# tux550/RayTracer-RPF

Hardware: AMD Instinct MI355X
Metric: RPF Msamples/sec filtered at 1080p×8spp (higher is better)
Workload: dtype f64

## Files before the change

### raytracer-rpf_amd/csrc/rpf_api.hip

```cpp
#include <hip/hip_runtime.h>
#include <dlfcn.h>

#include <chrono>
#include <climits>
#include <cmath>
#include <cstdio>
#include <cstdlib>
#include <cstring>
#include <string>
#include <thread>
#include <vector>

#include "rpf_internal.h"

using namespace rpf;

struct rpf_ctx {
    int device = 0;
    hipStream_t stream = nullptr;
    std::string err;
    char *d_planes = nullptr;    size_t cap_planes = 0;
    float *d_rayw = nullptr;     size_t cap_rayw = 0;
    double *d_colA = nullptr;    size_t cap_colA = 0;
    double *d_colB = nullptr;    size_t cap_colB = 0;
// ... 123 lines not shown
int32_t ensure_tables(rpf_ctx *ctx, int nmax) {
    if (ctx->d_tfix && ctx->tfix_n >= nmax + 1) return RPF_OK;
    std::vector<uint64_t> t((size_t)nmax + 1), d((size_t)nmax + 1, 0);
    t[0] = 0;
    for (int k = 1; k <= nmax; ++k) t[k] = (uint64_t)std::llroundl(std::ldexp((long double)k * std::log((long double)k), 44));
    for (int k = 0; k < nmax; ++k) d[k] = t[k + 1] - t[k];
    int32_t st;
    if ((st = ensure(ctx, ctx->d_tfix, ctx->cap_tfix, t.size() * sizeof(uint64_t)))) return st;
    if ((st = ensure(ctx, ctx->d_dfix, ctx->cap_dfix, d.size() * sizeof(uint64_t)))) return st;
    HIP_TRY(hipMemcpy(ctx->d_tfix, t.data(), t.size() * sizeof(uint64_t), hipMemcpyHostToDevice));
    HIP_TRY(hipMemcpy(ctx->d_dfix, d.data(), d.size() * sizeof(uint64_t), hipMemcpyHostToDevice));
    ctx->tfix_n = nmax + 1;
    return RPF_OK;
}

struct PassSetup {
    PassParams p;
    uint32_t lds = 0;
};

int32_t setup_pass(rpf_ctx *ctx, const rpf_desc *d, int box, const void *d_planes, const double *col_in,
                   double *col_out, const rpf_debug *dbg_dev, PassSetup &out) {
    if (box < 1 || (box & 1) == 0) return fail(ctx, RPF_E_BADARG, "box must be odd and positive");
    PassParams &p = out.p;
    std::memset(&p, 0, sizeof(p));
    p.W = d->W; p.H = d->H; p.S = d->S;
    p.lay = layout_of(d);
    const int kNFeat = p.lay.nF;
    p.row_begin = d->row_begin; p.row_end = d->row_end;
    p.box = box; p.b = (box - 1) / 2;
    p.beta_map = d->beta_map; p.policy = d->degenerate_policy;
    p.fast_weights = (d->flags & RPF_FLAG_FAST_WEIGHTS) ? 1 : 0;
    p.stage_mask = ctx->tun.stage_mask;
    p.screen = ctx->tun.screen;
    const int64_t nmax64 = (int64_t)box * box * d->S;
    if (nmax64 > kMaxNbhd) return fail(ctx, RPF_E_UNSUPPORTED, "box*box*S > 65535: neighbourhood too large (16-bit histogram cells, one-byte bin ids)");
    p.nmax = (int)nmax64;
    {
        const int64_t per_px = (int64_t)box * d->S * 88;
        const int64_t budget = d->S > 8 ? (256 << 10) : (1 << 20);
        int w = (int)(budget / std::max<int64_t>(per_px, 1)) - 2 * ((box - 1) / 2);
        w = std::max(8, std::min(128, w));
        p.strip_w = w & ~7;
        if (ctx->tun.strip_w > 0) p.strip_w = ctx->tun.strip_w;
    }
    p.bmax = (int)std::sqrt((double)p.nmax);
    if (p.bmax < 1) p.bmax = 1;
    p.eps = d->eps; p.seed = d->sigma_seed;
    p.sigma_p = (double)(box / 4);
    p.plane_stride = (uint64_t)d->W * d->H * d->S;
    p.planes = d_planes; p.col_in = col_in; p.col_out = col_out;
    const size_t HW = (size_t)d->W * d->H;
    int32_t st;
    if ((st = ensure(ctx, ctx->d_pmean, ctx->cap_pmean, HW * kNFeat * sizeof(double)))) return st;
    if ((st = ensure(ctx, ctx->d_pstd, ctx->cap_pstd, HW * kNFeat * sizeof(double)))) return st;
    if ((st = ensure(ctx, ctx->d_nbhd, ctx->cap_nbhd, HW * sizeof(int32_t)))) return st;
    if ((st = ensure_tables(ctx, p.nmax))) return st;
    p.pmean = ctx->d_pmean; p.pstd = ctx->d_pstd; p.tfix = ctx->d_tfix; p.dfix = ctx->d_dfix;
    p.nbhd = ctx->d_nbhd; p.status = ctx->d_status;
    if ((st = ensure(ctx, ctx->d_flat, ctx->cap_flat, HW))) return st;
    p.flat = ctx->d_flat; p.nan_flag = ctx->d_nan_flag;
    if (dbg_dev) p.dbg = *dbg_dev;
    {
        const int nres = std::min(p.nmax, kMaxResident), bres = std::max(1, (int)std::sqrt((double)nres));
        out.lds = lds_layout(p.S, nres, bres, table_in_lds(p.S, nres, bres, ctx->tun, p.lay), ctx->tun, p.lay).total;
    }
    if ((int)out.lds > max_lds_per_block())
// ... 590 lines not shown
    HIP_TRY(hipSetDevice(ctx->device));
    hipStream_t s = (hipStream_t)stream;
    return run_passes(ctx, d, d_planes, d_colour, s);
}

int32_t rpf_host_alloc(rpf_ctx *ctx, uint64_t bytes, void **out) {
    if (!ctx) return RPF_E_BADARG;
    if (!out) return fail(ctx, RPF_E_BADARG, "out is NULL");
    *out = nullptr;
    HIP_TRY(hipSetDevice(ctx->device));
    hipError_t e = hipHostMalloc(out, bytes ? (size_t)bytes : 16, hipHostMallocDefault);
    if (e != hipSuccess)
        return fail(ctx, e == hipErrorOutOfMemory ? RPF_E_NOMEM : RPF_E_HIP, std::string("hipHostMalloc: ") + hipGetErrorString(e));
    return RPF_OK;
}

int32_t rpf_host_free(rpf_ctx *ctx, void *ptr) {
    if (!ptr) return RPF_OK;
    const hipError_t e = hipHostFree(ptr);
    if (e != hipSuccess) return fail(ctx, RPF_E_HIP, std::string("hipHostFree: ") + hipGetErrorString(e));
    return RPF_OK;
}

int32_t rpf_set_option(rpf_ctx *ctx, const char *name, int64_t value) {
    if (!ctx) return RPF_E_BADARG;
    if (!name) return fail(ctx, RPF_E_BADARG, "option name is NULL");
    const std::string n(name);
    Tuning &t = ctx->tun;
    if (n == "stage_mask") t.stage_mask = (int32_t)value;
    else if (n == "binning" && value >= -1 && value <= 1) t.binning = (int32_t)value;
    else if (n == "waves_per_pixel" && (value == 0 || value == 1 || value == 4)) t.waves_per_pixel = (int32_t)value;
    else if (n == "table_in_lds" && value >= -1 && value <= 1) t.table_in_lds = (int32_t)value;
    else if (n == "screen" && value >= 0 && value <= 1) t.screen = (int32_t)value;
    else if (n == "split_weights" && value >= -1 && value <= 1) t.split_weights = (int32_t)value;
    else if (n == "strip_w" && value >= 0 && value <= 4096 && value % 8 == 0) t.strip_w = (int32_t)value;
    else if (n == "packed" && value >= -1 && value <= 1) t.packed = (int32_t)value;
    else if (n == "split_chunk" && value >= 0 && value <= (1 << 30)) t.split_chunk = (int32_t)value;
    else if (n == "count_first" && value >= -1 && value <= 1) t.count_first = (int32_t)value;
    else if (n == "lds_pad" && value >= 0 && value <= 160 * 1024) t.lds_pad = (int32_t)value;
    else return fail(ctx, RPF_E_BADARG, "unknown option or value out of range: " + n);
    ctx->bin_valid = false;
    return RPF_OK;
}

int32_t rpf_filter(rpf_ctx *ctx, const rpf_desc *d, const void *planes, const float *ray_weight,
                   float *sample_rgb_out, float *pixel_rgb_out) {
    return rpf_filter_ex(ctx, d, planes, nullptr, ray_weight, sample_rgb_out, pixel_rgb_out, nullptr);
}

int32_t rpf_filter_ex(rpf_ctx *ctx, const rpf_desc *d, const void *planes, const double *colour64_in,
                      const float *ray_weight, float *sample_rgb_out, float *pixel_rgb_out, double *colour64_out) {
    int32_t st = validate(ctx, d, true);
    if (st) return st;
    if (!planes) return fail(ctx, RPF_E_BADARG, "planes is NULL");
    HIP_TRY(hipSetDevice(ctx->device));
    hipStream_t s = ctx->stream;
    const size_t ps = (size_t)d->W * d->H * d->S, HW = (size_t)d->W * d->H;
    const SampleLayout lay = layout_of(d);
    const size_t plane_total = (size_t)lay.ndim() * ps * lay.plane_bytes();
    if ((st = ensure(ctx, ctx->d_planes, ctx->cap_planes, plane_total))) return st;
    if ((st = ensure(ctx, ctx->d_colA, ctx->cap_colA, 3 * ps * sizeof(double)))) return st;
    if (ray_weight && (st = ensure(ctx, ctx->d_rayw, ctx->cap_rayw, ps * sizeof(float)))) return st;
    if (sample_rgb_out && (st = ensure(ctx, ctx->d_srgb, ctx->cap_srgb, 3 * ps * sizeof(float)))) return st;
    if (pixel_rgb_out && (st = ensure(ctx, ctx->d_prgb, ctx->cap_prgb, 3 * HW * sizeof(float)))) return st;
    auto pinned = [](const void *p) {
        if (!p) return true;
// ... 567 lines not shown
```

### raytracer-rpf_amd/csrc/rpf_filter_impl.inc

```

constexpr int kNR = RPF_IMPL_NR;
constexpr int kNFeat = RPF_IMPL_NF;
constexpr int kColP = 0, kColC = 2, kColR = 5, kColF = 5 + kNR;
constexpr int kNDim = 5 + kNR + kNFeat;
constexpr int kNX = kNDim - 3;
constexpr int kNAnc = kNR + 2;
constexpr int kNPairF = kNFeat * kNAnc;
constexpr int kNPairC = kNAnc + kNFeat;
constexpr int kNPair = kNPairF + 3 * kNPairC;
#ifndef RPF_ROWS_EARLY
#define RPF_ROWS_EARLY 1
#endif
constexpr int kNWt = 5 + kNFeat;
constexpr bool kRef19 = (kNR == 2 && kNFeat == 12);
using plane_t = RPF_IMPL_PLANE_T;
static_assert(kNDim <= 32 && kNFeat <= 32, "lane maps: one chain lane per column inside a 32-lane half");

__host__ __device__ constexpr int xcol(int i) { return i < 2 ? i : i + 3; }
__device__ __forceinline__ float ldp(const PassParams &p, int col, uint32_t off) {
    return (float)reinterpret_cast<const plane_t *>(p.planes)[(uint64_t)col * p.plane_stride + off];
}
__device__ __forceinline__ void pair_cols(int pr, int &ca, int &cb) {
    if (pr < kNPairF) {
        const int i = pr / kNAnc, l = pr - i * kNAnc;
        ca = kColF + i;
        cb = l < kNR ? kColR + l : kColP + (l - kNR);
    } else {
        const int q = pr - kNPairF, c = q / kNPairC, l = q - c * kNPairC;
        ca = kColC + c;
        cb = l < kNR ? kColR + l : (l < kNAnc ? kColP + (l - kNR) : kColF + (l - kNAnc));
    }
}
__device__ __forceinline__ int pair_index_of(int a, int i) {
    return a < kNAnc ? (i < kNFeat ? i * kNAnc + a : kNPairF + (i - kNFeat) * kNPairC + a)
                     : kNPairF + (a - kNAnc) * kNPairC + kNAnc + i;
}
__device__ __forceinline__ int anchor_col(int a) { return a < kNR ? kColR + a : (a < kNAnc ? kColP + (a - kNR) : kColC + (a - kNAnc)); }

__device__ __forceinline__ double load_col(const PassParams &p, int c, uint32_t off) {
    if (c >= kColC && c < kColC + 3) return p.col_in[(uint64_t)(c - kColC) * p.plane_stride + off];
    return (double)ldp(p, c, off);
}
// ... 83 lines not shown
            if (KD > 12) reinterpret_cast<uint8_t *>(sBinW + kNDim * kWave * KW)[c * kWave + lane] = (uint8_t)b.b6;
        }
    }
}
template <int KD, int KW, int PACK5>
__device__ __forceinline__ void load_bins(const uint32_t *sBinW, int c, int lane, BinIds<KW, PACK5> &b) {
    if constexpr (PACK5 == 1) {
        b.w[0] = sBinW[c * kWave + lane];
        b.b6 = (KD > 6) ? (uint32_t) reinterpret_cast<const uint8_t *>(sBinW + kNDim * kWave)[c * kWave + lane] : 0u;
    } else {
        load_words<KW>(sBinW + ((size_t)c * kWave + lane) * KW, b.w);
        b.b6 = 0u;
        if constexpr (PACK5 == 7) {
            if (KD > 12) b.b6 = (uint32_t) reinterpret_cast<const uint8_t *>(sBinW + kNDim * kWave * KW)[c * kWave + lane];
        }
    }
}
template <int KW, int PACK5>
__device__ __forceinline__ uint32_t bin_of_sample(const uint32_t *sBinW, int c, int j) {
    const int ln = j & 63, slot = j >> 6;
    if constexpr (PACK5 == 1) {
        if (slot < 6) return (sBinW[c * kWave + ln] >> (5 * slot)) & 31u;
        return reinterpret_cast<const uint8_t *>(sBinW + kNDim * kWave)[c * kWave + ln];
    } else if constexpr (PACK5 == 7) {
        if (slot < 12) return (sBinW[((size_t)c * kWave + ln) * KW + slot / 6] >> (5 * (slot % 6))) & 31u;
        return reinterpret_cast<const uint8_t *>(sBinW + kNDim * kWave * KW)[c * kWave + ln];
    } else {
        constexpr int BITS = PACK5 == 6 ? 6 : 5, SPW = 32 / BITS;
        return (sBinW[((size_t)c * kWave + ln) * KW + slot / SPW] >> (BITS * (slot % SPW))) & ((1u << BITS) - 1u);
    }
}

constexpr int kColConst = 5;
__device__ __forceinline__ void column_constants(const double *sStat, double *sCK, int c) {
    const double Mc = sStat[c], SDc = sStat[kNDim + c];
    const double xlo = sStat[2 * kNDim + c], xhi = sStat[3 * kNDim + c];
    const bool sd0 = (SDc == 0.0);
    const UDiv dsd = udiv_prepare(SDc);
    const double lo = sd0 ? 0.0 : udiv(xlo - Mc, dsd);
    const double hi = sd0 ? 0.0 : udiv(xhi - Mc, dsd);
    const double range = hi - lo;
    const bool flat = !(hi != lo);
    const UDiv drg = udiv_prepare(range);
    const bool fast = dsd.fast && (flat || drg.fast);
    double *ck = sCK + c * kColConst;
    ck[0] = dsd.r; ck[1] = lo; ck[2] = range; ck[3] = drg.r;
    ck[4] = (double)((sd0 ? 1 : 0) | (flat ? 2 : 0) | (fast ? 4 : 0));
}

template <int KD, int KW, int PACK5, int NW = 1>
__device__ __forceinline__ void bins_stage(const PassParams &p, const double *sStat, const uint32_t *sOff, uint32_t *sBinW,
                                           int lane, int n, int B, const double *sCK, int wv = 0) {
    const double dB = (double)B;
    {
        uint32_t offk[KD];
#pragma unroll
        for (int kk = 0; kk < KD; ++kk) offk[kk] = (lane + kWave * kk < n) ? sOff[lane + kWave * kk] : 0u;
        auto do_column = [&](int c, const double (&xv)[KD]) {
            const double Mc = sStat[c], SDc = sStat[kNDim + c];
            const double *ck = sCK + c * kColConst;
            const double lo = ck[1], range = ck[2];
            const int flags = (int)ck[4];
            const bool sd0 = flags & 1, flat = flags & 2, fast = flags & 4;
            UDiv dsd, drg;
            dsd.b = SDc; dsd.r = ck[0]; dsd.fast = true;
            drg.b = range; drg.r = ck[3]; drg.fast = true;
            BinIds<KW, PACK5> w;
            w.clear();
            if (sd0 || flat) {
            } else if (fast) {
#pragma unroll
                for (int kk = 0; kk < KD; ++kk) {
                    const double a = xv[kk] - Mc;
                    const double z = udiv_fast(a, dsd);
                    const double t = udiv_fast(z - lo, drg) * dB;
                    int bin = (int)t;
                    bin = min(bin, B - 1);
                    bin = max(bin, 0);
                    bin = (lane + kWave * kk < n) ? bin : 0;
                    w.set(kk, (uint32_t)bin);
                }
            } else {
#pragma unroll
                for (int kk = 0; kk < KD; ++kk) {
                    if (lane + kWave * kk < n) {
                        const double a = xv[kk] - Mc;
                        const double z = sd0 ? 0.0 : a / SDc;
                        int bin = 0;
                        if (!flat) {
                            const double t = (z - lo) / range * dB;
                            bin = (int)t;
                            bin = min(bin, B - 1);
                            bin = max(bin, 0);
                        }
                        w.set(kk, (uint32_t)bin);
                    }
                }
            }
            store_bins<KD, KW, PACK5>(sBinW, c, lane, w);
        };
        if constexpr (NW > 1) {
            if (p.stage_mask & 2) {
                auto colidx = [](int i) { return xcol(i); };
                float xb[KD];
                auto issue3 = [&](int i) {
                    const plane_t *fplane = reinterpret_cast<const plane_t *>(p.planes) + (uint64_t)colidx(i) * p.plane_stride;
#pragma unroll
                    for (int kk = 0; kk < KD; ++kk) xb[kk] = (float)fplane[offk[kk]];
                };
                issue3(wv);
#pragma unroll 1
                for (int i = wv; i < kNX; i += NW) {
                    double xv[KD];
#pragma unroll
                    for (int kk = 0; kk < KD; ++kk) xv[kk] = (double)xb[kk];
                    if (i + NW < kNX) issue3(i + NW);
                    do_column(colidx(i), xv);
                }
#pragma unroll 1
                for (int c = wv; c < 3; c += NW) {
                    double xc[KD];
                    const double *dplane = p.col_in + (uint64_t)c * p.plane_stride;
#pragma unroll
                    for (int kk = 0; kk < KD; ++kk) xc[kk] = dplane[offk[kk]];
                    do_column(kColC + c, xc);
                }
            }
        } else if (p.stage_mask & 2) {
            constexpr int kPF3 = KD <= 8 ? 4 : (KD <= 13 ? 2 : 1);
            static_assert(kNX % 4 == 0, "the column loop below walks whole groups of kPF3");
            float xb[kPF3][KD];
            auto colidx = [](int i) { return xcol(i); };
            auto issue3 = [&](int i, float (&dst)[KD]) {
                const plane_t *fplane = reinterpret_cast<const plane_t *>(p.planes) + (uint64_t)colidx(i) * p.plane_stride;
#pragma unroll
                for (int kk = 0; kk < KD; ++kk) dst[kk] = (float)fplane[offk[kk]];
            };
#pragma unroll
            for (int u = 0; u < kPF3; ++u) issue3(u, xb[u]);
#pragma unroll 1
            for (int i0 = 0; i0 < kNX; i0 += kPF3) {
#pragma unroll
                for (int u = 0; u < kPF3; ++u) {
                    double xv[KD];
#pragma unroll
                    for (int kk = 0; kk < KD; ++kk) xv[kk] = (double)xb[u][kk];
                    if (i0 + u + kPF3 < kNX) issue3(i0 + u + kPF3, xb[u]);
                    do_column(colidx(i0 + u), xv);
                }
            }
            double xc[3][KD];
#pragma unroll
            for (int c = 0; c < 3; ++c) {
                const double *dplane = p.col_in + (uint64_t)c * p.plane_stride;
#pragma unroll
                for (int kk = 0; kk < KD; ++kk) xc[c][kk] = dplane[offk[kk]];
            }
#pragma unroll
            for (int c = 0; c < 3; ++c) do_column(kColC + c, xc[c]);
        }
    }
}

template <int NIT, bool ROWS>
__device__ __forceinline__ uint32_t marginal_counts(const uint32_t *sHist, int lane, int B) {
    uint32_t tot = 0u;
    const int j = lane & 31, h = lane >> 5;
    uint32_t v[NIT];
    if constexpr (!ROWS) {
        const uint32_t *col = sHist + h * B + j;
#pragma unroll
        for (int t = 0; t < NIT; ++t) v[t] = col[2 * t * B];
#pragma unroll
        for (int t = 0; t < NIT; ++t) tot += v[t];
    } else {
        const int jj = min(j, B - 1);
#pragma unroll
        for (int t = 0; t < NIT; ++t) v[t] = sHist[jj * B + min(2 * t + h, B - 1)];
#pragma unroll
// ... 835 lines not shown
                    for (int i = 0; i < 3; ++i) vd[i] = p.col_in[(uint64_t)i * p.plane_stride + off];
                }
            };
            fetch(lane);
            for (int j0 = 0; j0 < nrun; j0 += kStageChunk) {
                const int cnt = min(kStageChunk, nrun - j0);
                if (lane < cnt) {
#pragma unroll
                    for (int i = 0; i < kNX; ++i) {
                        fmn[i] = fminf(fmn[i], vf[i]);
                        fmx[i] = fmaxf(fmx[i], vf[i]);
                    }
#pragma unroll
                    for (int i = 0; i < 3; ++i) {
                        cmn[i] = fmin(cmn[i], vd[i]);
                        cmx[i] = fmax(cmx[i], vd[i]);
                    }
                    if (j0 + lane < S) {
#pragma unroll
                        for (int i = 0; i < kNX; ++i) sOwn[(j0 + lane) * kNDim + xcol(i)] = (double)vf[i];
#pragma unroll
                        for (int i = 0; i < 3; ++i) sOwn[(j0 + lane) * kNDim + kColC + i] = vd[i];
                    }
                }
#pragma unroll
                for (int hf = 0; hf < 2; ++hf) {
                    const int cnth = min(kStageHalf, cnt - hf * kStageHalf);
                    const int t = lane - hf * kStageHalf;
                    if (t >= 0 && t < cnth) {
#pragma unroll
                        for (int i = 0; i < kNX; ++i) sStage[xcol(i) * (kStageHalf + 1) + t] = (double)vf[i];
#pragma unroll
                        for (int i = 0; i < 3; ++i) sStage[(kColC + i) * (kStageHalf + 1) + t] = vd[i];
                    }
                    wsync();
                    if (hf == 1) fetch(j0 + kStageChunk + lane);
                    if (chain && cnth > 0) {
                        const double *src = sStage + myc * (kStageHalf + 1);
                        if (cnth == kStageHalf) {
#pragma unroll
                            for (int h = 0; h < kStageHalf; h += 16) {
                                double v[16];
#pragma unroll
                                for (int q = 0; q < 16; ++q) v[q] = src[h + q];
#pragma unroll
                                for (int q = 0; q < 16; ++q) v[q] = is_sq ? v[q] * v[q] : v[q];
#pragma unroll
                                for (int q = 0; q < 16; ++q) acc = acc + v[q];
                            }
                        } else if (!is_sq) {
                            for (int q = 0; q < cnth; ++q) acc = acc + src[q];
                        } else {
                            for (int q = 0; q < cnth; ++q) { const double v = src[q]; acc = acc + v * v; }
                        }
                    }
                    wsync();
                }
            }
            const double sq = __shfl(acc, (lane & 31) + 32, 64);
            const double dn = (double)n;
            const double mean = acc / dn;
            double sd = sqrt(sq / dn - mean * mean);
            if (p.policy == RPF_DEGEN_EPS && isnan(sd)) sd = 0.0;
            if (lane < kNDim) {
                sStat[lane] = mean;
                sStat[kNDim + lane] = sd;
                if (p.dbg.mean) p.dbg.mean[pix * kNDim + lane] = mean;
                if (p.dbg.stddev) p.dbg.stddev[pix * kNDim + lane] = sd;
            }
            {
                wave_minmax(fmn, fmx, lane, sStat + 2 * kNDim, sStat + 3 * kNDim);
#pragma unroll
                for (int i = 0; i < 3; ++i) {
                    const double lo = xl::allreduce<xl::OpMin>(cmn[i]), hi = xl::allreduce<xl::OpMax>(cmx[i]);
                    if (lane == 0) { sStat[2 * kNDim + kColC + i] = lo; sStat[3 * kNDim + kColC + i] = hi; }
                }
            }
            wsync();
        }

    }
    } else {
        bsync();
        const double *cr = p.carry + pix * kCarry;
        for (int k = tid; k < 4 * kNDim; k += kThreads) sStat[k] = cr[k];
        bsync();
    }
    if constexpr (PHASE == 3) {
        double *cw = p.carry + pix * kCarry;
        for (int k = tid; k < 4 * kNDim; k += kThreads) cw[k] = sStat[k];
        return;
    }

    const int B = max(1, (int)sqrt((double)n));
    const int kdyn = (n + kWave - 1) / kWave;
    double *sCK = reinterpret_cast<double *>(sPairF);
    if (tid < kNDim) column_constants(sStat, sCK, tid);
    bsync();
    if constexpr (K <= 8) {
        switch (kdyn) {
        case 1: bins_stage<1, KW, PACK5>(p, sStat, sOff, sBinW, lane, n, B, sCK); break;
        case 2: if constexpr (K >= 2) bins_stage<2, KW, PACK5>(p, sStat, sOff, sBinW, lane, n, B, sCK); break;
        case 3: if constexpr (K >= 3) bins_stage<3, KW, PACK5>(p, sStat, sOff, sBinW, lane, n, B, sCK); break;
        case 4: if constexpr (K >= 4) bins_stage<4, KW, PACK5>(p, sStat, sOff, sBinW, lane, n, B, sCK); break;
        case 5: if constexpr (K >= 5) bins_stage<5, KW, PACK5>(p, sStat, sOff, sBinW, lane, n, B, sCK); break;
        case 6: if constexpr (K >= 6) bins_stage<6, KW, PACK5>(p, sStat, sOff, sBinW, lane, n, B, sCK); break;
        case 7: if constexpr (K >= 7) bins_stage<7, KW, PACK5>(p, sStat, sOff, sBinW, lane, n, B, sCK); break;
        default: if constexpr (K >= 8) bins_stage<8, KW, PACK5>(p, sStat, sOff, sBinW, lane, n, B, sCK); break;
        }
    } else {
        bins_stage<K, KW, PACK5, NW>(p, sStat, sOff, sBinW, lane, n, B, sCK, wv);
    }
    bsync();
    if (p.dbg.bin_hash != nullptr && tid < kNDim) {
        uint32_t h = 2166136261u;
        for (int j = 0; j < n; ++j) h = fnv1a_u16(h, bin_of_sample<KW, PACK5>(sBinW, tid, j));
        p.dbg.bin_hash[pix * kNDim + tid] = h;
    }
    if (p.stage_mask & 4) {
        const uint64_t *dtab = T_IN_LDS ? sD : p.dfix;
        if constexpr (K <= 8 && kRef19) {
#define RPF_MI_CASE(KD_)                                                                                     \
    if constexpr (K >= KD_) {                                                                                \
        if constexpr (KD_ == 1) mi_stage_tiny<KW, PACK5>(sBinW, sHist, p.tfix, sHXf, sPairF, lane, n, B);  \
        else if constexpr (KD_ == 2) mi_stage_deep<KD_, KW, 1, PACK5>(sBinW, sHist, dtab, sHXf, sPairF, lane, n, B);  \
        else if (B * B <= 256) mi_pm<KD_, KW, 1, PACK5, !T_IN_LDS>(sBinW, sHist, dtab, sD0, p.tfix, sHXf, sPairF, lane, n, B); \
        else if (B * B <= 320) mi_pm<KD_, KW, 3, PACK5, !T_IN_LDS>(sBinW, sHist, dtab, sD0, p.tfix, sHXf, sPairF, lane, n, B); \
        else if (B * B <= 384) mi_pm<KD_, KW, 4, PACK5, !T_IN_LDS>(sBinW, sHist, dtab, sD0, p.tfix, sHXf, sPairF, lane, n, B); \
        else mi_pm<KD_, KW, 2, PACK5, !T_IN_LDS>(sBinW, sHist, dtab, sD0, p.tfix, sHXf, sPairF, lane, n, B);               \
    }
            switch (kdyn) {
            case 1: RPF_MI_CASE(1) break;
            case 2: RPF_MI_CASE(2) break;
            case 3: RPF_MI_CASE(3) break;
            case 4: RPF_MI_CASE(4) break;
            case 5: RPF_MI_CASE(5) break;
            case 6: RPF_MI_CASE(6) break;
            case 7: RPF_MI_CASE(7) break;
            default: RPF_MI_CASE(8) break;
            }
#undef RPF_MI_CASE
        } else {
            constexpr int kFullSlots = K == 13 ? 7 : (K == 25 ? 13 : (K == 49 ? 25 : 0));
            constexpr int kTSrc = T_IN_LDS ? 1 : 0;
// ... 315 lines not shown
                } else {
#pragma unroll
                for (int k = 0; k < kNWt; ++k) {
                    const double xv = k < 2 ? (double)pf[k] : (k < 5 ? pc[k < 5 && k >= 2 ? k - 2 : 0] : (double)pf[k >= 5 ? k - 3 : 0]);
                    const double z = sFastI[k] == 0.0 ? 0.0 : (xv - sFastM[k]) * sFastI[k];
                    zj[k] = z;
                    Bj = fma(sCoef[k] * z, z, Bj);
                }
                }
#pragma unroll
                for (int k = 0; k < 3; ++k) cj[k] = lane_ok ? pc[k] : 0.0;
                if constexpr (kAhead) fetch17(j + kWave);
                typedef float v2f __attribute__((ext_vector_type(2)));
                bool skip[kOwnBlock / 2];
#pragma unroll
                for (int pp = 0; pp < kOwnBlock / 2; ++pp) skip[pp] = false;
                if constexpr (kScreen) {
                    float zq[kQP];
#pragma unroll
                    for (int k = 0; k < kQP; ++k) zq[k] = k < kNWt ? (float)zj[k] : (k == kNWt ? 1.f : 0.f);
                    const double Bc = Bj + 0.0 * ((cj[0] + cj[1]) + cj[2]);
                    const float Bq = (Bc < 1e30) ? (float)(Bj * kScreenShrink - 747.0) : __builtin_nanf("");
#pragma unroll
                    for (int pp = 0; pp < kOwnBlock / 2; ++pp) {
                        const float4 *rq = reinterpret_cast<const float4 *>(sOwnQ + min((i0 >> 1) + pp, (S - 1) >> 1) * (kQP * 2));
                        v2f acc = {Bq, Bq};
#pragma unroll
                        for (int q = 0; q < kQP / 2; ++q) {
                            const float4 v = rq[q];
                            const v2f r0 = {v.x, v.y}, r1 = {v.z, v.w};
                            acc = __builtin_elementwise_fma(r0, (v2f)(zq[2 * q]), acc);
                            acc = __builtin_elementwise_fma(r1, (v2f)(zq[2 * q + 1]), acc);
                        }
                        skip[pp] = __all((acc.x > 0.f && acc.y > 0.f) || !lane_ok) && p.screen != 0;
                    }
                }
                double rowlo[kOwnBlock], rowhi[kNQ];
                asm volatile("" : "+v"(l16));
#pragma unroll
                for (int ii = 0; ii < kOwnBlock; ++ii) rowlo[ii] = sOwnU[min(i0 + ii, S - 1) * kOR + l16];
#pragma unroll
                for (int q = 0; q < kNQ; ++q) {
                    const int ii = min(q * kOwnsPerQ + l16 / kHiPad, kOwnBlock - 1);
                    rowhi[q] = sOwnU[min(i0 + ii, S - 1) * kOR + 16 + min(l16 % kHiPad, kRowHi - 1)];
                }
#if RPF_ROWS_EARLY
#pragma unroll
                for (int ii = 0; ii < kOwnBlock; ++ii) asm volatile("" : "+v"(rowlo[ii]));
#pragma unroll
                for (int q = 0; q < kNQ; ++q) asm volatile("" : "+v"(rowhi[q]));
#endif
                auto exponent = [&](auto iic) -> double {
                    constexpr int ii = decltype(iic)::value;
                    constexpr int qi = ii / kOwnsPerQ, qb = (ii % kOwnsPerQ) * kHiPad;
                    double e0 = xl::rowbc<qb + (kNWt - 16), true>(rowhi[qi]) + Bj, e1 = 0.0, e2 = 0.0, e3 = 0.0;
                    xl::static_for<0, kNWt>([&](auto kc) {
                        constexpr int k = decltype(kc)::value;
                        double &e = (k >= kW4 || (k & 3) == 0) ? e0 : ((k & 3) == 1 ? e1 : ((k & 3) == 2 ? e2 : e3));
                        if constexpr (k < 16) xl::fmac_rowbc<k>(e, rowlo[ii], zj[k]);
                        else xl::fmac_rowbc<qb + (k - 16)>(e, rowhi[qi], zj[k]);
                    });
                    return (e0 + e1) + (e2 + e3);
                };
                auto weigh = [&](auto iic, double E) {
                    constexpr int ii = decltype(iic)::value;
                    double w = exp(-E);
                    w = lane_ok ? w : 0.0;
                    sw[ii] += w;
                    s0[ii] = fma(w, cj[0], s0[ii]);
                    s1[ii] = fma(w, cj[1], s1[ii]);
                    s2[ii] = fma(w, cj[2], s2[ii]);
                };
                if constexpr (kEVote) {
                    double Ev[kOwnBlock];
                    xl::static_for<0, kOwnBlock>([&](auto iic) { Ev[decltype(iic)::value] = exponent(iic); });
                    bool far = (0.0 * ((cj[0] + cj[1]) + cj[2])) == 0.0;
#pragma unroll
                    for (int ii = 0; ii < kOwnBlock; ++ii) far = far && (Ev[ii] > 746.0);
                    if (p.screen != 0 && __all(far || !lane_ok)) continue;
                    xl::static_for<0, kOwnBlock>([&](auto iic) { weigh(iic, Ev[decltype(iic)::value]); });
                } else {
                    xl::static_for<0, kOwnBlock>([&](auto iic) {
                        if (skip[decltype(iic)::value >> 1]) return;
                        weigh(iic, exponent(iic));
                    });
                }
            }
        } else {
#pragma unroll 1
            for (int kk = 0; kk < K; ++kk) {
                const int j = lane + kWave * kk;
                if (j >= n) break;
                if constexpr (!kAhead) fetch17(j);
                float zj[kNWt];
                double cj[3];
                zj[0] = (float)(((double)pf[0] - sFastM[0]) * sFastI[0]);
                zj[1] = (float)(((double)pf[1] - sFastM[1]) * sFastI[1]);
#pragma unroll
                for (int k = 0; k < 3; ++k) { cj[k] = pc[k]; zj[2 + k] = (float)((pc[k] - sFastM[2 + k]) * sFastI[2 + k]); }
#pragma unroll
                for (int k = 0; k < kNFeat; ++k) zj[5 + k] = (float)(((double)pf[2 + k] - sFastM[5 + k]) * sFastI[5 + k]);
#pragma unroll
                for (int k = 0; k < kNWt; ++k)
                    if (sFastI[k] == 0.0) zj[k] = 0.f;
                if constexpr (kAhead) fetch17(j + kWave);
#pragma unroll
                for (int ii = 0; ii < kOwnBlock; ++ii) {
                    const int i = i0 + ii;
                    if (i < S) {
                        const float *zi = sFastZ + i * kFZ;
                        float zo[kFZ];
#pragma unroll
// ... 680 lines not shown
```

### raytracer-rpf_amd/csrc/rpf_internal.h

```cpp
#pragma once
#include <hip/hip_runtime.h>
#include <stdint.h>

#include "rpf_hip.h"

namespace rpf {

constexpr int kWave = 64;

struct SampleLayout {
    int32_t nR = 2, nF = 12, f16 = 0;
    int ndim() const { return 5 + nR + nF; }
    int npair() const { return nF * (nR + 2) + 3 * (nR + 2 + nF); }
    int nwt() const { return 5 + nF; }
    size_t plane_bytes() const { return f16 ? 2 : 4; }
    bool is_ref19() const { return nR == 2 && nF == 12 && !f16; }
    bool supported() const { return is_ref19() || (nR == 4 && nF == 18 && f16 == 1); }
};
constexpr int kStageChunk = 64;
constexpr int kStageHalf = 32;

struct PassParams {
    int32_t W, H, S;
    int32_t row_begin, row_end;
// ... 7 lines not shown
    int32_t bmax;
    double eps, seed, sigma_p;
    uint64_t plane_stride;
    SampleLayout lay;
    const void *planes;
    const double *col_in;
    double *col_out;
    const double *pmean;
    const double *pstd;
    const uint64_t *tfix;
    const uint64_t *dfix;
    int32_t *nbhd;
    double *carry;
    const uint32_t *pix_list;
    uint32_t list_count;
    uint64_t *masks;
    uint32_t mask_stride;
    uint64_t *reroute_masks;
    uint8_t *flat;
    int32_t *nan_flag;
    uint32_t *redo_list;
    uint32_t *redo_count;
    int32_t *status;
    rpf_debug dbg;
};

struct Tuning {
    int32_t waves_per_pixel = 0;
    int32_t table_in_lds = -1;
    int32_t lds_pad = 0;
    int32_t binning = -1;
    int32_t stage_mask = -1;
    int32_t screen = 1;
    int32_t split_weights = -1;
    int32_t split_chunk = 0;
    int32_t strip_w = 0;
    int32_t count_first = -1;
    int32_t packed = -1;
    bool is_default() const { return waves_per_pixel == 0 && table_in_lds == -1 && lds_pad == 0 && binning == -1 && stage_mask == -1 && screen == 1 && strip_w == 0 && split_chunk == 0 && count_first == -1 && split_weights == -1 && packed == -1; }
};

struct LdsLayout {
    uint32_t off_T, off_stat, off_hx, off_pair, off_mi, off_own, off_off, off_union, off_hist, total;
    uint32_t hist_stride;
    uint32_t nw;
};
LdsLayout lds_layout(int S, int nmax, int bmax, bool t_in_lds, const Tuning &tun, const SampleLayout &lay);
LdsLayout lds_layout_weights(int S, int nmax, const SampleLayout &lay, int nw);
LdsLayout lds_layout_chains(int S, int nmax, const SampleLayout &lay, int nw);
constexpr int kCarryStride = 136;
int samples_per_lane(int nmax);
bool table_in_lds(int S, int nmax, int bmax, const Tuning &tun, const SampleLayout &lay);
int waves_per_pixel(int nmax, const Tuning &tun);

hipError_t launch_pixel_stats(const PassParams &p, hipStream_t s);
hipError_t launch_pixel_stats_rows(const PassParams &p, int r0, int r1, hipStream_t s);
hipError_t launch_filter_pass(const PassParams &p, const Tuning &tun, hipStream_t s, uint32_t *lds_bytes_out);
constexpr int kNumPacked = 4;
constexpr int kNumClasses = 11;
constexpr int kMaxResident = 3136;
constexpr int kMaxNbhd = 65535;
int class_capacity(int c);
hipError_t launch_filter_packed(const PassParams &p, int lanes_per_pixel, const uint32_t *count_dev, hipStream_t s);
hipError_t launch_nbhd_count(const PassParams &p, int step, uint32_t *probe, const uint32_t *list, const uint32_t *list_count,
                             uint32_t list_max, hipStream_t s);
hipError_t launch_filter_big(const PassParams &p, void *list, void *bins, uint32_t slots, const uint32_t *count_dev, hipStream_t s);
hipError_t launch_classify(const PassParams &p, uint32_t *lists , uint32_t *counts ,
                           int max_class, int rest_class, hipStream_t s);
hipError_t launch_colour_from_planes(const void *planes, bool f16, double *colour, uint64_t plane_stride, hipStream_t s);
hipError_t launch_colour_from_planes_span(const void *planes, bool f16, double *colour, uint64_t plane_stride, uint64_t e0,
                                          uint64_t cnt, hipStream_t s);
hipError_t launch_copy_f64(const double *src, double *dst, uint64_t n, hipStream_t s);
// ... 30 lines not shown
```

### raytracer-rpf_amd/csrc/rpf_xlane.h

```cpp
#pragma once
#include <hip/hip_runtime.h>
#include <stdint.h>
#include <type_traits>

namespace rpf {
namespace xl {

constexpr int kQuadXor1 = 0xB1;
constexpr int kQuadXor2 = 0x4E;
constexpr int kRowMirror = 0x140;
constexpr int kRowHalfMirror = 0x141;

struct OpSum {
    template <class T> __device__ __forceinline__ static T f(T a, T b) { return a + b; }
};
struct OpMin {
    __device__ __forceinline__ static float f(float a, float b) { return fminf(a, b); }
    __device__ __forceinline__ static double f(double a, double b) { return fmin(a, b); }
};
struct OpMax {
    __device__ __forceinline__ static float f(float a, float b) { return fmaxf(a, b); }
    __device__ __forceinline__ static double f(double a, double b) { return fmax(a, b); }
};

// ... 126 lines not shown
    for (int i = 0; i < 2; ++i) b2[i] = exch_row<Op, kRowHalfMirror, 4>(b4[i], b4[i + 2], lane);
    const T v = exch_row<Op, kQuadXor2, 2>(b2[0], b2[1], lane);
    return allreduce_bit0<Op>(v);
}

template <int I, int N, class F>
__device__ __forceinline__ void static_for(F &&f) {
    if constexpr (I < N) {
        f(std::integral_constant<int, I>{});
        static_for<I + 1, N>(f);
    }
}

template <int N, bool NOP = false>
__device__ __forceinline__ void fmac_rowbc(double &acc, double row, double z) {
    static_assert(N >= 0 && N < 16, "lane of a 16-lane row");
    if constexpr (NOP)
        asm("s_nop 1\n\tv_fmac_f64_dpp %0, %1, %2 row_newbcast:%3 row_mask:0xf bank_mask:0xf" : "+v"(acc) : "v"(row), "v"(z), "n"(N));
    else
        asm("v_fmac_f64_dpp %0, %1, %2 row_newbcast:%3 row_mask:0xf bank_mask:0xf" : "+v"(acc) : "v"(row), "v"(z), "n"(N));
}

template <int N, bool NOP = false>
__device__ __forceinline__ double rowbc(double row) {
    static_assert(N >= 0 && N < 16, "lane of a 16-lane row");
    double out;
    if constexpr (NOP)
        asm("s_nop 1\n\tv_mov_b64_dpp %0, %1 row_newbcast:%2 row_mask:0xf bank_mask:0xf" : "=v"(out) : "v"(row), "n"(N));
    else
        asm("v_mov_b64_dpp %0, %1 row_newbcast:%2 row_mask:0xf bank_mask:0xf" : "=v"(out) : "v"(row), "n"(N));
    return out;
}

}
}
```

Measured before the change: 264.5.

## Screen histogram bin assignment in fp32 with error-bounded fallback to exact fp64

Per column, the code precomputes an fp32 slope/offset and a rigorous rounding-error bound (delta). Bin indices are then computed in fp32 for each wave, and the exact fp64 double-divide path is rerun only when some live lane lands within delta of a bin boundary. This replaces most fp64 divides in the binning stage with cheap fp32 math while keeping results identical, at the cost of extra LDS for screen constants and a ballot per column. It also restructures the staged column-sum loop into 8-wide blocks that square only the upper half-wave through an exec-masked asm helper, padding partial chunks with -0.0 so the loop can stay vectorised.

New measurement: 266.9, median of 6. About the same (+0.9%).

```diff
diff --git a/raytracer-rpf_amd/csrc/rpf_api.hip b/raytracer-rpf_amd/csrc/rpf_api.hip
--- a/raytracer-rpf_amd/csrc/rpf_api.hip
+++ b/raytracer-rpf_amd/csrc/rpf_api.hip
@@ -179,7 +179,7 @@
     p.beta_map = d->beta_map; p.policy = d->degenerate_policy;
     p.fast_weights = (d->flags & RPF_FLAG_FAST_WEIGHTS) ? 1 : 0;
     p.stage_mask = ctx->tun.stage_mask;
-    p.screen = ctx->tun.screen;
+    p.screen = (ctx->tun.screen ? 1 : 0) | (ctx->tun.bin_screen ? 0 : 2);
     const int64_t nmax64 = (int64_t)box * box * d->S;
     if (nmax64 > kMaxNbhd) return fail(ctx, RPF_E_UNSUPPORTED, "box*box*S > 65535: neighbourhood too large (16-bit histogram cells, one-byte bin ids)");
     p.nmax = (int)nmax64;
@@ -836,6 +836,7 @@
     else if (n == "waves_per_pixel" && (value == 0 || value == 1 || value == 4)) t.waves_per_pixel = (int32_t)value;
     else if (n == "table_in_lds" && value >= -1 && value <= 1) t.table_in_lds = (int32_t)value;
     else if (n == "screen" && value >= 0 && value <= 1) t.screen = (int32_t)value;
+    else if (n == "bin_screen" && value >= 0 && value <= 1) t.bin_screen = (int32_t)value;
     else if (n == "split_weights" && value >= -1 && value <= 1) t.split_weights = (int32_t)value;
     else if (n == "strip_w" && value >= 0 && value <= 4096 && value % 8 == 0) t.strip_w = (int32_t)value;
     else if (n == "packed" && value >= -1 && value <= 1) t.packed = (int32_t)value;
diff --git a/raytracer-rpf_amd/csrc/rpf_filter_impl.inc b/raytracer-rpf_amd/csrc/rpf_filter_impl.inc
--- a/raytracer-rpf_amd/csrc/rpf_filter_impl.inc
+++ b/raytracer-rpf_amd/csrc/rpf_filter_impl.inc
@@ -8,6 +8,17 @@
 constexpr int kNPairF = kNFeat * kNAnc;
 constexpr int kNPairC = kNAnc + kNFeat;
 constexpr int kNPair = kNPairF + 3 * kNPairC;
+#ifdef RPF_BIN_SCREEN_STATS
+static __device__ unsigned long long g_bin_screen_stats[2];
+#if RPF_IMPL_PART == 1 && RPF_IMPL_NR == 2 && RPF_IMPL_NF == 12
+extern "C" int rpf_bin_screen_stats(unsigned long long *out2, int reset) {
+    const unsigned long long zero[2] = {0ull, 0ull};
+    hipError_t e = hipMemcpyFromSymbol(out2, HIP_SYMBOL(g_bin_screen_stats), sizeof(zero));
+    if (e == hipSuccess && reset) e = hipMemcpyToSymbol(HIP_SYMBOL(g_bin_screen_stats), zero, sizeof(zero));
+    return (int)e;
+}
+#endif
+#endif
 #ifndef RPF_ROWS_EARLY
 #define RPF_ROWS_EARLY 1
 #endif
@@ -157,7 +168,11 @@
 }
 
 constexpr int kColConst = 5;
-__device__ __forceinline__ void column_constants(const double *sStat, double *sCK, int c) {
+constexpr int kScreenMaxKD = 25;
+struct ColFlags { int32_t flags; float delta; };
+struct ColScreen { float xlo, slope; };
+static_assert(sizeof(ColFlags) == 8 && sizeof(ColScreen) == 8, "one 8-byte slot each");
+__device__ __forceinline__ void column_constants(const double *sStat, double *sCK, ColScreen *sSC, int c, int B, bool screen_on) {
     const double Mc = sStat[c], SDc = sStat[kNDim + c];
     const double xlo = sStat[2 * kNDim + c], xhi = sStat[3 * kNDim + c];
     const bool sd0 = (SDc == 0.0);
@@ -168,24 +183,42 @@
     const bool flat = !(hi != lo);
     const UDiv drg = udiv_prepare(range);
     const bool fast = dsd.fast && (flat || drg.fast);
+    const double dB = (double)B;
+    const double S1 = dB / SDc / range;
+    const double X = fmax(fabs(xlo), fabs(xhi)), Zm = fmax(fabs(lo), fabs(hi));
+    const bool colour = c >= kColC && c < kColC + 3;
+    const double delta = 3.5 * 0x1p-24 * (dB + 1.0)
+                         + (colour ? 2.5 * 0x1p-24 * X * S1 : 0.0)
+                         + 0x1p-50 * dB * (1.0 + Zm / range)
+                         + 0x1p-100 * (1.0 + S1);
+    const bool proof = screen_on && fast && !sd0 && !flat && SDc > 0.0 && range > 0.0 && xlo <= xhi && X < 0x1p100 &&
+                       Zm < 0x1p100 && S1 > 0x1p-100 && S1 < 0x1p100 && delta < 0.125;
     double *ck = sCK + c * kColConst;
     ck[0] = dsd.r; ck[1] = lo; ck[2] = range; ck[3] = drg.r;
-    ck[4] = (double)((sd0 ? 1 : 0) | (flat ? 2 : 0) | (fast ? 4 : 0));
-}
-
-template <int KD, int KW, int PACK5, int NW = 1>
+    ColFlags cf;
+    cf.flags = (sd0 ? 1 : 0) | (flat ? 2 : 0) | (fast ? 4 : 0) | (proof ? 8 : 0);
+    cf.delta = (float)(delta * 1.000001);
+    *reinterpret_cast<ColFlags *>(ck + 4) = cf;
+    ColScreen sc;
+    sc.xlo = (float)xlo;
+    sc.slope = (float)S1;
+    sSC[c] = sc;
+}
+
+template <int KD, int KW, int PACK5, int NW = 1, bool FRONTFULL = false>
 __device__ __forceinline__ void bins_stage(const PassParams &p, const double *sStat, const uint32_t *sOff, uint32_t *sBinW,
-                                           int lane, int n, int B, const double *sCK, int wv = 0) {
+                                           int lane, int n, int B, const double *sCK, const ColScreen *sSC, int wv = 0) {
     const double dB = (double)B;
     {
         uint32_t offk[KD];
 #pragma unroll
         for (int kk = 0; kk < KD; ++kk) offk[kk] = (lane + kWave * kk < n) ? sOff[lane + kWave * kk] : 0u;
-        auto do_column = [&](int c, const double (&xv)[KD]) {
+        auto do_column = [&](int c, const auto &xin) {
             const double Mc = sStat[c], SDc = sStat[kNDim + c];
             const double *ck = sCK + c * kColConst;
             const double lo = ck[1], range = ck[2];
-            const int flags = (int)ck[4];
+            const ColFlags cf = *reinterpret_cast<const ColFlags *>(ck + 4);
+            const int flags = cf.flags;
             const bool sd0 = flags & 1, flat = flags & 2, fast = flags & 4;
             UDiv dsd, drg;
             dsd.b = SDc; dsd.r = ck[0]; dsd.fast = true;
@@ -194,22 +227,49 @@
             w.clear();
             if (sd0 || flat) {
             } else if (fast) {
-#pragma unroll
-                for (int kk = 0; kk < KD; ++kk) {
-                    const double a = xv[kk] - Mc;
-                    const double z = udiv_fast(a, dsd);
-                    const double t = udiv_fast(z - lo, drg) * dB;
-                    int bin = (int)t;
-                    bin = min(bin, B - 1);
-                    bin = max(bin, 0);
-                    bin = (lane + kWave * kk < n) ? bin : 0;
-                    w.set(kk, (uint32_t)bin);
+                bool exact = true;
+                if ((flags & 8) && KD <= kScreenMaxKD) {
+                    const ColScreen sc = sSC[c];
+                    const float hiB = (float)B - 0.5f;
+                    float dmin = 0.5f;
+#pragma unroll
+                    for (int kk = 0; kk < KD; ++kk) {
+                        const float te = ((float)xin[kk] - sc.xlo) * sc.slope;
+                        const float tc = __builtin_amdgcn_fmed3f(te, 0.5f, hiB);
+                        const float d = fabsf(tc - rintf(tc));
+                        if (FRONTFULL && kk < KD - 1) {
+                            dmin = fminf(dmin, d);
+                            w.set(kk, (uint32_t)(int)tc);
+                        } else {
+                            const bool live = lane + kWave * kk < n;
+                            dmin = fminf(dmin, live ? d : 0.5f);
+                            w.set(kk, live ? (uint32_t)(int)tc : 0u);
+                        }
+                    }
+                    exact = __builtin_amdgcn_ballot_w64(!(dmin > cf.delta)) != 0;
+#ifdef RPF_BIN_SCREEN_STATS
+                    if (lane == 0) atomicAdd(&g_bin_screen_stats[exact ? 1 : 0], 1ull);
+#endif
+                }
+                if (exact) {
+                    w.clear();
+#pragma unroll
+                    for (int kk = 0; kk < KD; ++kk) {
+                        const double a = (double)xin[kk] - Mc;
+                        const double z = udiv_fast(a, dsd);
+                        const double t = udiv_fast(z - lo, drg) * dB;
+                        int bin = (int)t;
+                        bin = min(bin, B - 1);
+                        bin = max(bin, 0);
+                        bin = (lane + kWave * kk < n) ? bin : 0;
+                        w.set(kk, (uint32_t)bin);
+                    }
                 }
             } else {
 #pragma unroll
                 for (int kk = 0; kk < KD; ++kk) {
                     if (lane + kWave * kk < n) {
-                        const double a = xv[kk] - Mc;
+                        const double a = (double)xin[kk] - Mc;
                         const double z = sd0 ? 0.0 : a / SDc;
                         int bin = 0;
                         if (!flat) {
@@ -236,9 +296,9 @@
                 issue3(wv);
 #pragma unroll 1
                 for (int i = wv; i < kNX; i += NW) {
-                    double xv[KD];
-#pragma unroll
-                    for (int kk = 0; kk < KD; ++kk) xv[kk] = (double)xb[kk];
+                    float xv[KD];
+#pragma unroll
+                    for (int kk = 0; kk < KD; ++kk) xv[kk] = xb[kk];
                     if (i + NW < kNX) issue3(i + NW);
                     do_column(colidx(i), xv);
                 }
@@ -267,9 +327,9 @@
             for (int i0 = 0; i0 < kNX; i0 += kPF3) {
 #pragma unroll
                 for (int u = 0; u < kPF3; ++u) {
-                    double xv[KD];
-#pragma unroll
-                    for (int kk = 0; kk < KD; ++kk) xv[kk] = (double)xb[u][kk];
+                    float xv[KD];
+#pragma unroll
+                    for (int kk = 0; kk < KD; ++kk) xv[kk] = xb[u][kk];
                     if (i0 + u + kPF3 < kNX) issue3(i0 + u + kPF3, xb[u]);
                     do_column(colidx(i0 + u), xv);
                 }
@@ -1171,26 +1231,40 @@
                         for (int i = 0; i < kNX; ++i) sStage[xcol(i) * (kStageHalf + 1) + t] = (double)vf[i];
 #pragma unroll
                         for (int i = 0; i < 3; ++i) sStage[(kColC + i) * (kStageHalf + 1) + t] = vd[i];
+                    } else if (t >= 0 && t >= cnth && t < ((cnth + 7) & ~7)) {
+#pragma unroll
+                        for (int c = 0; c < kNDim; ++c) sStage[c * (kStageHalf + 1) + t] = -0.0;
                     }
                     wsync();
                     if (hf == 1) fetch(j0 + kStageChunk + lane);
                     if (chain && cnth > 0) {
                         const double *src = sStage + myc * (kStageHalf + 1);
+                        auto load8 = [&](int h, double (&v)[8]) {
+#pragma unroll
+                            for (int q = 0; q < 8; ++q) v[q] = src[h + q];
+                        };
+                        auto sum8 = [&](double (&v)[8]) {
+                            xl::square8_if(v, 0xffffffff00000000ull);
+#pragma unroll
+                            for (int q = 0; q < 8; ++q) acc = acc + v[q];
+                        };
                         if (cnth == kStageHalf) {
-#pragma unroll
-                            for (int h = 0; h < kStageHalf; h += 16) {
-                                double v[16];
-#pragma unroll
-                                for (int q = 0; q < 16; ++q) v[q] = src[h + q];
-#pragma unroll
-                                for (int q = 0; q < 16; ++q) v[q] = is_sq ? v[q] * v[q] : v[q];
-#pragma unroll
-                                for (int q = 0; q < 16; ++q) acc = acc + v[q];
+                            double va[8], vb[8];
+                            load8(0, va);
+                            load8(8, vb);
+                            sum8(va);
+                            load8(16, va);
+                            sum8(vb);
+                            load8(24, vb);
+                            sum8(va);
+                            sum8(vb);
+                        } else {
+#pragma unroll 1
+                            for (int h = 0; h < cnth; h += 8) {
+                                double v[8];
+                                load8(h, v);
+                                sum8(v);
                             }
-                        } else if (!is_sq) {
-                            for (int q = 0; q < cnth; ++q) acc = acc + src[q];
-                        } else {
-                            for (int q = 0; q < cnth; ++q) { const double v = src[q]; acc = acc + v * v; }
                         }
                     }
                     wsync();
@@ -1234,21 +1308,22 @@
     const int B = max(1, (int)sqrt((double)n));
     const int kdyn = (n + kWave - 1) / kWave;
     double *sCK = reinterpret_cast<double *>(sPairF);
-    if (tid < kNDim) column_constants(sStat, sCK, tid);
+    ColScreen *sSC = reinterpret_cast<ColScreen *>(sHXf);
+    if (tid < kNDim) column_constants(sStat, sCK, sSC, tid, B, (p.screen & 2) == 0);
     bsync();
     if constexpr (K <= 8) {
         switch (kdyn) {
-        case 1: bins_stage<1, KW, PACK5>(p, sStat, sOff, sBinW, lane, n, B, sCK); break;
-        case 2: if constexpr (K >= 2) bins_stage<2, KW, PACK5>(p, sStat, sOff, sBinW, lane, n, B, sCK); break;
-        case 3: if constexpr (K >= 3) bins_stage<3, KW, PACK5>(p, sStat, sOff, sBinW, lane, n, B, sCK); break;
-        case 4: if constexpr (K >= 4) bins_stage<4, KW, PACK5>(p, sStat, sOff, sBinW, lane, n, B, sCK); break;
-        case 5: if constexpr (K >= 5) bins_stage<5, KW, PACK5>(p, sStat, sOff, sBinW, lane, n, B, sCK); break;
-        case 6: if constexpr (K >= 6) bins_stage<6, KW, PACK5>(p, sStat, sOff, sBinW, lane, n, B, sCK); break;
-        case 7: if constexpr (K >= 7) bins_stage<7, KW, PACK5>(p, sStat, sOff, sBinW, lane, n, B, sCK); break;
-        default: if constexpr (K >= 8) bins_stage<8, KW, PACK5>(p, sStat, sOff, sBinW, lane, n, B, sCK); break;
+        case 1: bins_stage<1, KW, PACK5, 1, true>(p, sStat, sOff, sBinW, lane, n, B, sCK, sSC); break;
+        case 2: if constexpr (K >= 2) bins_stage<2, KW, PACK5, 1, true>(p, sStat, sOff, sBinW, lane, n, B, sCK, sSC); break;
+        case 3: if constexpr (K >= 3) bins_stage<3, KW, PACK5, 1, true>(p, sStat, sOff, sBinW, lane, n, B, sCK, sSC); break;
+        case 4: if constexpr (K >= 4) bins_stage<4, KW, PACK5, 1, true>(p, sStat, sOff, sBinW, lane, n, B, sCK, sSC); break;
+        case 5: if constexpr (K >= 5) bins_stage<5, KW, PACK5, 1, true>(p, sStat, sOff, sBinW, lane, n, B, sCK, sSC); break;
+        case 6: if constexpr (K >= 6) bins_stage<6, KW, PACK5, 1, true>(p, sStat, sOff, sBinW, lane, n, B, sCK, sSC); break;
+        case 7: if constexpr (K >= 7) bins_stage<7, KW, PACK5, 1, true>(p, sStat, sOff, sBinW, lane, n, B, sCK, sSC); break;
+        default: if constexpr (K >= 8) bins_stage<8, KW, PACK5, 1, true>(p, sStat, sOff, sBinW, lane, n, B, sCK, sSC); break;
         }
     } else {
-        bins_stage<K, KW, PACK5, NW>(p, sStat, sOff, sBinW, lane, n, B, sCK, wv);
+        bins_stage<K, KW, PACK5, NW>(p, sStat, sOff, sBinW, lane, n, B, sCK, sSC, wv);
     }
     bsync();
     if (p.dbg.bin_hash != nullptr && tid < kNDim) {
@@ -1630,7 +1705,7 @@
                             acc = __builtin_elementwise_fma(r0, (v2f)(zq[2 * q]), acc);
                             acc = __builtin_elementwise_fma(r1, (v2f)(zq[2 * q + 1]), acc);
                         }
-                        skip[pp] = __all((acc.x > 0.f && acc.y > 0.f) || !lane_ok) && p.screen != 0;
+                        skip[pp] = __all((acc.x > 0.f && acc.y > 0.f) || !lane_ok) && (p.screen & 1) != 0;
                     }
                 }
                 double rowlo[kOwnBlock], rowhi[kNQ];
@@ -1675,7 +1750,7 @@
                     bool far = (0.0 * ((cj[0] + cj[1]) + cj[2])) == 0.0;
 #pragma unroll
                     for (int ii = 0; ii < kOwnBlock; ++ii) far = far && (Ev[ii] > 746.0);
-                    if (p.screen != 0 && __all(far || !lane_ok)) continue;
+                    if ((p.screen & 1) != 0 && __all(far || !lane_ok)) continue;
                     xl::static_for<0, kOwnBlock>([&](auto iic) { weigh(iic, Ev[decltype(iic)::value]); });
                 } else {
                     xl::static_for<0, kOwnBlock>([&](auto iic) {
diff --git a/raytracer-rpf_amd/csrc/rpf_internal.h b/raytracer-rpf_amd/csrc/rpf_internal.h
--- a/raytracer-rpf_amd/csrc/rpf_internal.h
+++ b/raytracer-rpf_amd/csrc/rpf_internal.h
@@ -63,12 +63,13 @@
     int32_t binning = -1;
     int32_t stage_mask = -1;
     int32_t screen = 1;
+    int32_t bin_screen = 1;
     int32_t split_weights = -1;
     int32_t split_chunk = 0;
     int32_t strip_w = 0;
     int32_t count_first = -1;
     int32_t packed = -1;
-    bool is_default() const { return waves_per_pixel == 0 && table_in_lds == -1 && lds_pad == 0 && binning == -1 && stage_mask == -1 && screen == 1 && strip_w == 0 && split_chunk == 0 && count_first == -1 && split_weights == -1 && packed == -1; }
+    bool is_default() const { return waves_per_pixel == 0 && table_in_lds == -1 && lds_pad == 0 && binning == -1 && stage_mask == -1 && screen == 1 && bin_screen == 1 && strip_w == 0 && split_chunk == 0 && count_first == -1 && split_weights == -1 && packed == -1; }
 };
 
 struct LdsLayout {
diff --git a/raytracer-rpf_amd/csrc/rpf_xlane.h b/raytracer-rpf_amd/csrc/rpf_xlane.h
--- a/raytracer-rpf_amd/csrc/rpf_xlane.h
+++ b/raytracer-rpf_amd/csrc/rpf_xlane.h
@@ -182,5 +182,15 @@
     return out;
 }
 
+__device__ __forceinline__ void square8_if(double (&v)[8], uint64_t mask) {
+    uint64_t saved;
+    asm("s_and_saveexec_b64 %8, %9\n\t"
+        "v_mul_f64 %0, %0, %0\n\tv_mul_f64 %1, %1, %1\n\tv_mul_f64 %2, %2, %2\n\tv_mul_f64 %3, %3, %3\n\t"
+        "v_mul_f64 %4, %4, %4\n\tv_mul_f64 %5, %5, %5\n\tv_mul_f64 %6, %6, %6\n\tv_mul_f64 %7, %7, %7\n\t"
+        "s_mov_b64 exec, %8"
+        : "+v"(v[0]), "+v"(v[1]), "+v"(v[2]), "+v"(v[3]), "+v"(v[4]), "+v"(v[5]), "+v"(v[6]), "+v"(v[7]), "=&s"(saved)
+        : "s"(mask) : "scc");
+}
+
 }
 }
```
